# zhongzisha/multi_frame_super_resolution

Measured on AMD Instinct MI355X. Metric: Mpix/s end-to-end (N-frame burst -> x2 SR), higher is better.
Workload: dtype f32

## Files before the change

### include/mfsr.h

```cpp
#ifndef MFSR_H
#define MFSR_H

#include <stddef.h>
#include <stdint.h>

#ifdef __cplusplus
extern "C" {
#endif

#define MFSR_VERSION 100
#define MFSR_MAX_FUSE_GROUP 4

typedef void* mfsr_stream_t;

typedef struct { float x, y; } mfsr_float2;
typedef struct { float x, y, z; } mfsr_float3;
typedef struct { float x, y, z, w; } mfsr_float4;

typedef struct {
    const void* ptr;
    int32_t pitch;
    int32_t width;
    int32_t height;
} mfsr_tex2d;
// ... 228 lines not shown
                                    const float* movedImg, int pitchImg, const float* sumIn, const float* diffIn, float* sumOut,
                                    float* diffOut, int pitchSD, int width, int height, int halfWindowSize, float minDet,
                                    float outScale, mfsr_stream_t stream);
typedef struct {
    const uint16_t* dataIn;
    mfsr_float3* halfOut;
    float* pyr0;
    float* pyr1;
} mfsr_prepare_frame;
int mfsr_prepareFrameFusedBatch(int nFrames, const mfsr_prepare_frame* frames, int halfPitch, float maxVal, int dimX, int dimY,
                                int pyr0Pitch, int pyr1Pitch, const float* taps, int ntaps, mfsr_stream_t stream);
typedef struct {
    const float* movedImg;
    const mfsr_float2* coarseShifts;
    mfsr_float2* coordinates;
    const mfsr_prealign* base;
} mfsr_track_frame;
int mfsr_trackTilesFastSupported(int tileSize, int maxShift);
int mfsr_trackTilesFusedBatch(int nFrames, const mfsr_track_frame* frames, const float* refImg, int coarsePitch, int oldLevel,
                              int newLevel, int oldCountX, int oldCountY, int oldTileSize, int coordinatesPitch, int imgWidth,
                              int imgHeight, int imgPitch, int maxShift, int tileSize, int tileCountX, int tileCountY, float threshold,
                              const float* refSquaredSums, float baseInvScale, mfsr_stream_t stream);
typedef struct {
    mfsr_float2* outImg;
    const mfsr_float2* tileShifts;
    const mfsr_prealign* base;
    const float* movedImg;
    float* sumOut;
    float* diffOut;
} mfsr_flowfield_frame;
int mfsr_CreateFlowFieldWarpedBatch(int nFrames, const mfsr_flowfield_frame* frames, int tilePitch, int tileCountX, int tileCountY,
                                    int imgWidth, int imgHeight, int imgPitch, const float* refImg, int pitchImg, int pitchSD,
                                    mfsr_stream_t stream);
typedef struct {
    const mfsr_float3* movedHalf;
    mfsr_float4* mask;
    const mfsr_float2* flow;
} mfsr_robustness_frame;
int mfsr_robustnessMaskFusedBatch(int nFrames, const mfsr_robustness_frame* frames, const mfsr_float3* rawImgRef, int flowPitch,
                                  int flowWidth, int flowHeight, int imgWidth, int imgHeight, int imgPitch, int maskPitch, float alpha,
                                  float beta, float thresholdM, mfsr_stream_t stream);
typedef struct {
    const mfsr_float2* shiftsIn;
    mfsr_float2* shiftsOut;
    const float* movedImg;
    const float* sumIn;
    const float* diffIn;
    float* sumOut;
    float* diffOut;
} mfsr_lk_frame;
int mfsr_lucasKanadeSweepBatch(int nFrames, const mfsr_lk_frame* frames, const float* refImg, int pitchShift, int pitchImg,
                               int pitchSD, int width, int height, int halfWindowSize, float minDet, float outScale,
                               mfsr_stream_t stream);
int mfsr_CreateFlowFieldWarped(mfsr_float2* outImg, mfsr_tex2d texObjShiftXY, int imgWidth, int imgHeight, int imgPitch,
                               mfsr_float2 baseShift, float baseRotation, const mfsr_prealign* base, const float* refImg,
                               const float* movedImg, int pitchImg, float* sumOut, float* diffOut, int pitchSD,
                               mfsr_stream_t stream);

int mfsr_finishFusedRows(const mfsr_float3* finalImg, const mfsr_float3* weight, int imgPitch, const mfsr_float3* fallback,
                         int fbPitch, int fbW, int fbH, float u0, float u1, float v0, float v1, mfsr_float3* outImg,
                         int outPitch, uint16_t* out16, int width, int height, float threshold, int applyGamma, float maxOut,
                         int rowOffset, int fullHeight, mfsr_stream_t stream);
int mfsr_finishFusedWindow(const mfsr_float3* finalImg, const mfsr_float3* weight, int imgPitch, const mfsr_float3* fallback,
                           int fbPitch, int fbW, int fbH, float u0, float u1, float v0, float v1, mfsr_float3* outImg,
                           int outPitch, uint16_t* out16, int width, int height, float threshold, int applyGamma, float maxOut,
                           int colOffset, int rowOffset, int fullWidth, int fullHeight, mfsr_stream_t stream);

typedef struct {
    int32_t width, height;
    int32_t frames;
    int32_t reference;
    int32_t scale;
    int32_t mono;
    int32_t cfa[4];
    float black[3], white[3];
    float maxVal;
    int32_t levels;
    int32_t levelFactor[4];
    int32_t tileSize[4];
    int32_t maxShift[4];
    float minimumThreshold;
    float sigmaTracking;
    int32_t lkIterations;
    int32_t lkHalfWindow;
    float lkMinDet;
    float alpha, beta, thresholdM;
    float sigmaTensor;
    float Dth, Dtr, kDetail, kDenoise, kStretch, kShrink;
    float weightThreshold;
    int32_t applyGamma;
    int32_t fused;
    int32_t pairFrames;
    int32_t asyncFuse;
    int32_t preAlign;
    float preAlignMaxAngle;
    int32_t uploadRing;
    int32_t reserved[2];
} mfsr_config;

typedef struct mfsr_burst mfsr_burst;

int mfsr_config_default(mfsr_config* cfg, int width, int height, int frames, int scale, int mono);
size_t mfsr_burst_workspace_bytes(const mfsr_config* cfg);
size_t mfsr_burst_accumulator_bytes(const mfsr_config* cfg);
int mfsr_burst_create(mfsr_burst** out, const mfsr_config* cfg, void* workspace, size_t workspaceBytes);
void mfsr_burst_destroy(mfsr_burst* b);
// ... 87 lines not shown
```

### multi_frame_super_resolution_amd/csrc/lk_fused.hip

```cpp
#include <cstdlib>
#include <cstring>
#include "common.hpp"
#include "lk_math.hpp"

#ifndef LK_TY
#define LK_TY 16
#endif

__device__ __forceinline__ int lk_mirror_index(int i, int n)
{
    i = i < 0 ? -1 - i : i;
    return i >= n ? 2 * n - 1 - i : i;
}

template <typename T>
__device__ __forceinline__ T* lk_at(T* base, int pitch, int y, int x)
{
    return (T*)((char*)base + (uint32_t)((uint32_t)y * (uint32_t)pitch + (uint32_t)x * (uint32_t)sizeof(T)));
}

__device__ __forceinline__ void lk_warp_sample(const float* __restrict__ refImg, const float* __restrict__ movedImg, int pitchImg,
                                               int width, int height, int gx, int gy, float2 f, float& wv, float& rv,
                                               const MfsrExactDiv* dW = nullptr, const MfsrExactDiv* dH = nullptr)
{
// ... 231 lines not shown
            }                                                                                                          \
        }                                                                                                              \
        hipLaunchKernelGGL((k_lkIterationFused<HT, TXV, PRE>), grid, block, lds, mfsr_s(stream), (const float2*)shiftsIn, \
                           (float2*)shiftsOut, pitchShift, refImg, movedImg, pitchImg, width, height, h, minDet,       \
                           outScale, sumIn, diffIn, sumOut, diffOut, pitchSD);                                         \
    } while (0)
#define LK_CASE(HT)                                                                                                    \
    case HT:                                                                                                           \
        if (PRE && TX == 64)                                                                                           \
            LK_LAUNCH(HT, 64);                                                                                         \
        else if (TX == 48)                                                                                             \
            LK_LAUNCH(HT, 48);                                                                                         \
        else                                                                                                           \
            LK_LAUNCH(HT, 32);                                                                                         \
        break;
    switch (h) {
        LK_CASE(1)
        LK_CASE(2)
        LK_CASE(3)
        LK_CASE(4)
        LK_CASE(5)
        LK_CASE(6)
        LK_CASE(7)
        default:
            if (TX != 32) return MFSR_E_UNSUPPORTED;
            LK_LAUNCH(0, 32);
            break;
    }
#undef LK_CASE
#undef LK_LAUNCH
    return mfsr_launch_status("lucasKanadeIterationFused");
}

extern "C" int mfsr_lucasKanadeIterationFused(const mfsr_float2* shiftsIn, mfsr_float2* shiftsOut, int pitchShift,
                                              const float* refImg, const float* movedImg, int pitchImg, int width,
                                              int height, int halfWindowSize, float minDet, float outScale, mfsr_stream_t stream)
{
    return lk_iteration_impl<false>(shiftsIn, shiftsOut, pitchShift, refImg, movedImg, pitchImg, width, height, halfWindowSize, minDet,
                                    outScale, nullptr, nullptr, nullptr, nullptr, 0, stream);
}

extern "C" int mfsr_lucasKanadeIterationWarped(const mfsr_float2* shiftsIn, mfsr_float2* shiftsOut, int pitchShift,
                                               const float* refImg, const float* movedImg, int pitchImg, const float* sumIn,
                                               const float* diffIn, float* sumOut, float* diffOut, int pitchSD, int width, int height,
                                               int halfWindowSize, float minDet, float outScale, mfsr_stream_t stream)
{
    MFSR_REQUIRE(sumIn && diffIn && (sumOut != nullptr) == (diffOut != nullptr) && sumOut != sumIn && diffOut != diffIn);
    MFSR_REQUIRE((long long)pitchSD >= 4LL * width && (pitchSD & 3) == 0);
    MFSR_REQUIRE(!sumOut || outScale == 1.0f);
    return lk_iteration_impl<true>(shiftsIn, shiftsOut, pitchShift, refImg, movedImg, pitchImg, width, height, halfWindowSize, minDet,
                                   outScale, sumIn, diffIn, sumOut, diffOut, pitchSD, stream);
}

template <bool BASE_PTR>
__global__ void __launch_bounds__(256)
    k_flowFieldWarped(float2* __restrict__ outImg, mfsr_tex2d texShift, int imgWidth, int imgHeight, int imgPitch, float2 baseShift,
                      float baseRotation, const mfsr_prealign* __restrict__ base, const float* __restrict__ refImg,
                      const float* __restrict__ movedImg, int pitchImg, float* __restrict__ sumOut, float* __restrict__ diffOut,
                      int pitchSD, MfsrBatch bt, MfsrExactDiv dW, MfsrExactDiv dH)
{
    if (gridDim.z > 1) {
        outImg = (float2*)bt.p[blockIdx.z][0];
        texShift.ptr = bt.p[blockIdx.z][1];
        base = (const mfsr_prealign*)bt.p[blockIdx.z][2];
        movedImg = (const float*)bt.p[blockIdx.z][3];
        sumOut = (float*)bt.p[blockIdx.z][4];
        diffOut = (float*)bt.p[blockIdx.z][5];
    }
    const int pxX = blockIdx.x * blockDim.x + threadIdx.x;
    const int pxY = blockIdx.y * blockDim.y + threadIdx.y;
    if (pxX >= imgWidth || pxY >= imgHeight) return;
    float cf = 1.0f, sf = 0.0f, bx, by;
    if (BASE_PTR) {
        cf = base->cosRotation;
        sf = base->sinRotation;
        bx = base->shiftX;
        by = base->shiftY;
    } else {
        if (baseRotation != 0.0f) {
            cf = cosf(baseRotation);
            sf = sinf(baseRotation);
        }
        bx = baseShift.x;
        by = baseShift.y;
    }
    float2 shift;
    shift.x = cf * -bx - sf * -by;
    shift.y = sf * -bx + cf * -by;
    const float patchCenterX = (float)(pxX - imgWidth / 2);
    const float patchCenterY = (float)(pxY - imgHeight / 2);
    shift.x += cf * patchCenterX - sf * patchCenterY - patchCenterX;
    shift.y += sf * patchCenterX + cf * patchCenterY - patchCenterY;
    const float2 shiftPatch =
        tex2<ADDR_CLAMP>(texShift, mfsr_div((float)pxX + 0.5f, dW), mfsr_div((float)pxY + 0.5f, dH));
    shift.x += shiftPatch.x;
    shift.y += shiftPatch.y;
    *lk_at(outImg, imgPitch, pxY, pxX) = shift;
    float wv, rv;
    lk_warp_sample(refImg, movedImg, pitchImg, imgWidth, imgHeight, pxX, pxY, shift, wv, rv, &dW, &dH);
    *lk_at(sumOut, pitchSD, pxY, pxX) = wv + rv;
    *lk_at(diffOut, pitchSD, pxY, pxX) = wv - rv;
}

static int flow_field_warped_impl(int n, const mfsr_flowfield_frame* f, int tilePitch, int tileW, int tileH, int imgWidth, int imgHeight,
                                  int imgPitch, mfsr_float2 baseShift, float baseRotation, const float* refImg, int pitchImg, int pitchSD,
                                  mfsr_stream_t stream)
{
    MFSR_REQUIRE(f && n >= 1 && n <= MFSR_BATCH_MAX && refImg && imgWidth >= 2 && imgHeight >= 2);
    MFSR_REQUIRE((long long)imgPitch >= 8LL * imgWidth && (imgPitch & 7) == 0);
    MFSR_REQUIRE((long long)pitchImg >= 4LL * imgWidth && (pitchImg & 3) == 0 && (long long)pitchSD >= 4LL * imgWidth && (pitchSD & 3) == 0);
    if ((long long)imgPitch * imgHeight >= (1LL << 32) || (long long)pitchImg * imgHeight >= (1LL << 32) ||
        (long long)pitchSD * imgHeight >= (1LL << 32))
        return MFSR_E_UNSUPPORTED;
    mfsr_tex2d tex;
    tex.ptr = f[0].tileShifts;
    tex.pitch = tilePitch;
    tex.width = tileW;
    tex.height = tileH;
    MFSR_REQUIRE(mfsr_tex_ok(tex, 8) && (tilePitch & 7) == 0);
    MfsrBatch bt;
    memset(&bt, 0, sizeof(bt));
    for (int i = 0; i < n; i++) {
        MFSR_REQUIRE(f[i].outImg && f[i].tileShifts && f[i].movedImg && f[i].sumOut && f[i].diffOut);
        MFSR_REQUIRE(((uintptr_t)f[i].outImg & 7) == 0 && ((uintptr_t)f[i].tileShifts & 7) == 0);
        MFSR_REQUIRE((f[i].base != nullptr) == (f[0].base != nullptr));
        bt.p[i][0] = f[i].outImg;
        bt.p[i][1] = f[i].tileShifts;
        bt.p[i][2] = f[i].base;
        bt.p[i][3] = f[i].movedImg;
        bt.p[i][4] = f[i].sumOut;
        bt.p[i][5] = f[i].diffOut;
    }
    dim3 block(64, 4), grid(mfsr_cdiv(imgWidth, 64), mfsr_cdiv(imgHeight, 4), n);
    const MfsrExactDiv dW = mfsr_exact_div((float)imgWidth), dH = mfsr_exact_div((float)imgHeight);
    if (f[0].base)
        hipLaunchKernelGGL(k_flowFieldWarped<true>, grid, block, 0, mfsr_s(stream), (float2*)f[0].outImg, tex, imgWidth, imgHeight, imgPitch,
                           make_float2(0.0f, 0.0f), 0.0f, f[0].base, refImg, f[0].movedImg, pitchImg, f[0].sumOut, f[0].diffOut, pitchSD, bt, dW, dH);
    else
        hipLaunchKernelGGL(k_flowFieldWarped<false>, grid, block, 0, mfsr_s(stream), (float2*)f[0].outImg, tex, imgWidth, imgHeight, imgPitch,
                           make_float2(baseShift.x, baseShift.y), baseRotation, f[0].base, refImg, f[0].movedImg, pitchImg, f[0].sumOut,
                           f[0].diffOut, pitchSD, bt, dW, dH);
    return mfsr_launch_status("CreateFlowFieldWarped");
}

extern "C" int mfsr_CreateFlowFieldWarped(mfsr_float2* outImg, mfsr_tex2d texObjShiftXY, int imgWidth, int imgHeight, int imgPitch,
                                          mfsr_float2 baseShift, float baseRotation, const mfsr_prealign* base, const float* refImg,
                                          const float* movedImg, int pitchImg, float* sumOut, float* diffOut, int pitchSD,
                                          mfsr_stream_t stream)
{
    const mfsr_flowfield_frame f = {outImg, (const mfsr_float2*)texObjShiftXY.ptr, base, movedImg, sumOut, diffOut};
    return flow_field_warped_impl(1, &f, texObjShiftXY.pitch, texObjShiftXY.width, texObjShiftXY.height, imgWidth, imgHeight, imgPitch,
                                  baseShift, baseRotation, refImg, pitchImg, pitchSD, stream);
}

extern "C" int mfsr_CreateFlowFieldWarpedBatch(int nFrames, const mfsr_flowfield_frame* frames, int tilePitch, int tileCountX,
                                               int tileCountY, int imgWidth, int imgHeight, int imgPitch, const float* refImg,
                                               int pitchImg, int pitchSD, mfsr_stream_t stream)
{
    const mfsr_float2 z = {0.0f, 0.0f};
    return flow_field_warped_impl(nFrames, frames, tilePitch, tileCountX, tileCountY, imgWidth, imgHeight, imgPitch, z, 0.0f, refImg,
                                  pitchImg, pitchSD, stream);
}

#define MFSR_LK_SWEEP_MAX_BATCH 4
struct LkSweepFrame {
    const float2* flowIn;
    float2* flowOut;
    const float* moved;
    const float* sumIn;
    const float* diffIn;
    float* sumOut;
    float* diffOut;
};
struct LkSweepBatch {
    LkSweepFrame f[MFSR_LK_SWEEP_MAX_BATCH];
};

__device__ __forceinline__ float lk_wshr1(float v)
{
    return __uint_as_float(__builtin_amdgcn_update_dpp(0u, __float_as_uint(v), 0x138, 0xf, 0xf, true));
}
__device__ __forceinline__ float lk_wshl1(float v)
{
    return __uint_as_float(__builtin_amdgcn_update_dpp(0u, __float_as_uint(v), 0x130, 0xf, 0xf, true));
}

#ifndef LK_RV_REREAD
#define LK_RV_REREAD 0
#endif
#ifndef LK_DIFF_LATE
#define LK_DIFF_LATE 1
#endif
struct LkGather {
    float t00, t10, t01, t11, a, b;
#if !LK_RV_REREAD
    float rv;
#endif
};
__device__ __forceinline__ void lk_warp_issue(const float* __restrict__ movedImg, int pitchImg, int width, int height, int gx, int gy,
                                              float2 f, bool wanted, LkGather& g, const MfsrExactDiv& dW, const MfsrExactDiv& dH)
{
    const float u = mfsr_div((float)gx + 0.5f + f.x, dW);
    const float v = mfsr_div((float)gy + 0.5f + f.y, dH);
    const float xB = u * (float)width - 0.5f, yB = v * (float)height - 0.5f;
    const float fx = floorf(xB), fy = floorf(yB);
    const int ix = f2i(fx), iy = f2i(fy);
    const bool interior = u >= 0.0f && u < 1.0f && v >= 0.0f && v < 1.0f && (uint32_t)ix <= (uint32_t)(width - 2) &&
                          (uint32_t)iy <= (uint32_t)(height - 2);
    const int ixc = clampi(ix, 0, width - 2), iyc = clampi(iy, 0, height - 2);
    const float* r0 = lk_at(movedImg, pitchImg, iyc, ixc);
    const float* r1 = lk_at(movedImg, pitchImg, iyc + 1, ixc);
    g.t00 = r0[0], g.t10 = r0[1], g.t01 = r1[0], g.t11 = r1[1];
    g.a = xB - fx, g.b = yB - fy;
    if (__ballot(!interior && wanted) != 0) {
        mfsr_tex2d texMoved;
        texMoved.ptr = movedImg;
        texMoved.pitch = pitchImg;
        texMoved.width = width;
        texMoved.height = height;
        const float full = tex1<ADDR_MIRROR>(texMoved, u, v);
        if (!interior) {
            g.t00 = g.t10 = g.t01 = g.t11 = full;
            g.a = g.b = 0.0f;
        }
    }
}
__device__ __forceinline__ float lk_warp_finish(const LkGather& g) { return lerp4(g.t00, g.t10, g.t01, g.t11, g.a, g.b); }

template <int HT>
__global__ void __launch_bounds__(64)
    k_lkSweep(LkSweepBatch batch, const float* __restrict__ refImg, int pitchShift, int pitchImg, int pitchSD, int width, int height,
              float minDet, float outScale, int bandRows, int strips, int bands, int perXcd, int nFramesLaunch, MfsrExactDiv dW, MfsrExactDiv dH)
{
    constexpr int h = HT, HALO = HT + 2, WIN = 2 * HT + 1, VW = 64 - 2 * HALO;
    int sIdx, bIdx, fIdx;
    if (perXcd > 0) {
        const int t = ((int)blockIdx.x & 7) * perXcd + ((int)blockIdx.x >> 3);
        if (t >= strips * bands * nFramesLaunch) return;
        sIdx = t % strips;
        bIdx = (t / strips) % bands;
        fIdx = t / (strips * bands);
    } else {
        sIdx = blockIdx.x, bIdx = blockIdx.y, fIdx = blockIdx.z;
    }
    const LkSweepFrame F = batch.f[fIdx];
    const int lane = threadIdx.x;
    const int cx0 = sIdx * VW, ry0 = bIdx * bandRows;
    const int colIn = cx0 - HALO + lane;
    const int gxIn = lk_mirror_index(colIn, width);
    const int colOut = colIn - h;
    const bool outLane = lane >= 2 * h + 2 && lane <= 61 && colOut < width;
    const int colOutC = min(max(colOut, 0), width - 1);
    const bool ringCol = colOut < h || colOut >= width - h;
    const int rows = min(bandRows, height - ry0);
    const int T = rows + 2 * HALO;

    float s0 = 0, s1 = 0, s2 = 0, s3 = 0, s4 = 0;
    float d0 = 0;
    float H[5][WIN];
#pragma unroll
    for (int k = 0; k < 5; k++)
#pragma unroll
        for (int j = 0; j < WIN; j++) H[k][j] = 0.0f;

    auto load_sum = [&](int t, float& sv) { sv = *lk_at(F.sumIn, pitchSD, lk_mirror_index(ry0 - HALO + t, height), gxIn); };
    auto load_diff = [&](int t, float& dv) { dv = *lk_at(F.diffIn, pitchSD, lk_mirror_index(ry0 - HALO + t, height), gxIn); };
    float sA, sB, dA = 0, dB = 0;
    load_sum(0, sA);
    load_sum(min(1, T - 1), sB);
#if !LK_DIFF_LATE
    float d1 = 0, d2 = 0;
    load_diff(0, dA);
    load_diff(min(1, T - 1), dB);
#endif
    LkGather pend;
    int pendY = -1;
    auto finish_pending = [&]() {
        if (pendY < 0) return;
        const float wv = lk_warp_finish(pend);
#if LK_RV_REREAD
        const float rv = *lk_at(refImg, pitchImg, pendY, colOutC);
#else
        const float rv = pend.rv;
#endif
        if (outLane) {
            *lk_at(F.sumOut, pitchSD, pendY, colOutC) = wv + rv;
            *lk_at(F.diffOut, pitchSD, pendY, colOutC) = wv - rv;
        }
    };

    for (int t0 = 0; t0 < T; t0 += WIN) {
#pragma unroll
        for (int j = 0; j < WIN; j++) {
            const int t = t0 + j;
            if (t >= T) break;
            s0 = s1, s1 = s2, s2 = s3, s3 = s4, s4 = sA;
#if LK_DIFF_LATE
            d0 = dA, dA = dB;
            sA = sB;
            load_sum(min(t + 2, T - 1), sB);
            load_diff(t, dB);
#else
            d0 = d1, d1 = d2, d2 = dA, dA = dB;
            sA = sB;
            load_sum(min(t + 2, T - 1), sB);
            load_diff(min(t + 2, T - 1), dB);
#endif
            if (t < 4) continue;
            const int y = ry0 + t - 2 * HALO;
            const int yc = min(max(y, 0), height - 1);
            float2 shift = *lk_at(F.flowIn, pitchShift, yc, colOutC);
#if !LK_RV_REREAD
            const float rvOwn = *lk_at(refImg, pitchImg, yc, colOutC);
#endif
            const float xp1 = lk_wshl1(s2), xp2 = lk_wshl1(xp1), xm1 = lk_wshr1(s2), xm2 = lk_wshr1(xm1);
            float tx = xp2;
            tx -= xp1 * 8.0f;
            tx += xm1 * 8.0f;
            tx -= xm2;
            const float Ix = tx * (1.0f / 24.0f);
            float ty = s4;
            ty -= s3 * 8.0f;
            ty += s1 * 8.0f;
            ty -= s0;
            const float Iy = ty * (1.0f / 24.0f);
            const float It = d0;
            float P[5] = {Ix * Ix, Ix * Iy, Iy * Iy, Ix * It, Iy * It};
#pragma unroll
            for (int k = 0; k < 5; k++) {
                float acc = P[k];
#pragma unroll
                for (int q = 0; q < 2 * HT; q++) acc = P[k] + lk_wshr1(acc);
                H[k][j] = acc;
            }
            if (t < 2 * HALO) continue;
            float V[5];
#pragma unroll
            for (int k = 0; k < 5; k++) {
                float sum = 0;
#pragma unroll
                for (int d = 1; d <= WIN; d++) sum += H[k][(j + d) % WIN];
                V[k] = sum;
            }
            if (!(ringCol || y < h || y >= height - h)) {
                float inv[4];
                if (lk_pinv(V[0], V[1], V[2], minDet, inv)) {
                    float UV0 = inv[0] * V[3] + inv[1] * V[4];
                    float UV1 = inv[2] * V[3] + inv[3] * V[4];
                    UV0 = isnan(UV0) ? 0 : UV0;
                    UV1 = isnan(UV1) ? 0 : UV1;
                    shift.x += UV0;
                    shift.y += UV1;
                }
            }
            if (F.sumOut) {
                finish_pending();
                lk_warp_issue(F.moved, pitchImg, width, height, colOutC, y, shift, outLane, pend, dW, dH);
#if !LK_RV_REREAD
                pend.rv = rvOwn;
#endif
                pendY = y;
            }
            shift.x *= outScale;
            shift.y *= outScale;
            if (outLane) *lk_at(F.flowOut, pitchShift, y, colOutC) = shift;
        }
    }
    if (F.sumOut) finish_pending();
}

extern "C" int mfsr_lucasKanadeSweepBatch(int nFrames, const mfsr_lk_frame* frames, const float* refImg, int pitchShift, int pitchImg,
                                          int pitchSD, int width, int height, int halfWindowSize, float minDet, float outScale,
                                          mfsr_stream_t stream)
{
    MFSR_REQUIRE(frames && refImg && nFrames >= 1 && nFrames <= MFSR_LK_SWEEP_MAX_BATCH);
    if (halfWindowSize < 1 || halfWindowSize > 7 || width < 64 || height < 2 * (halfWindowSize + 2)) return MFSR_E_UNSUPPORTED;
    MFSR_REQUIRE((long long)pitchShift >= 8LL * width && (pitchShift & 7) == 0);
    MFSR_REQUIRE((long long)pitchImg >= 4LL * width && (pitchImg & 3) == 0 && (long long)pitchSD >= 4LL * width && (pitchSD & 3) == 0);
    if ((long long)pitchShift * height >= (1LL << 32) || (long long)pitchImg * height >= (1LL << 32) || (long long)pitchSD * height >= (1LL << 32))
        return MFSR_E_UNSUPPORTED;
    LkSweepBatch b;
    memset(&b, 0, sizeof(b));
    for (int i = 0; i < nFrames; i++) {
        const mfsr_lk_frame& f = frames[i];
        MFSR_REQUIRE(f.shiftsIn && f.shiftsOut && f.shiftsIn != f.shiftsOut && f.movedImg && f.sumIn && f.diffIn);
        MFSR_REQUIRE(((uintptr_t)f.shiftsIn & 7) == 0 && ((uintptr_t)f.shiftsOut & 7) == 0);
        MFSR_REQUIRE((f.sumOut != nullptr) == (f.diffOut != nullptr) && f.sumOut != f.sumIn && f.diffOut != f.diffIn);
        MFSR_REQUIRE(!f.sumOut || outScale == 1.0f);
        b.f[i] = LkSweepFrame{(const float2*)f.shiftsIn, (float2*)f.shiftsOut, f.movedImg, f.sumIn, f.diffIn, f.sumOut, f.diffOut};
    }
    const int h = halfWindowSize, VW = 64 - 2 * (h + 2);
    const int strips = mfsr_cdiv(width, VW);
    static const int forceBand = [] {
        const char* e = getenv("MFSR_LK_BAND");
        return e ? atoi(e) : 0;
    }();
    int band = (int)((long long)height * strips * nFrames / 8192);
    band = (band + 4) & ~7;
    band = band < 8 ? 8 : (band > 32 ? 32 : band);
    {
        static const int occ[8] = {0, 8, 7, 6, 5, 4, 4, 4};
        const long long places = 1024LL * occ[h];
        const long long maxBands = places / ((long long)strips * nFrames);
        if (maxBands >= 1) {
            int b = (int)((height + maxBands - 1) / maxBands);
            b = b < 8 ? 8 : b;
            if (b <= 64) band = b;
        }
    }
    if (forceBand >= 8) band = forceBand;
    static const int xcdRemap = [] {
        const char* e = getenv("MFSR_LK_XCD");
        return e ? atoi(e) : 1;
    }();
    const int bands = mfsr_cdiv(height, band);
    const int total = strips * bands * nFrames;
    const int perXcd = xcdRemap ? mfsr_cdiv(total, 8) : 0;
    dim3 grid = perXcd ? dim3(8 * perXcd, 1, 1) : dim3(strips, bands, nFrames), block(64);
    const MfsrExactDiv dW = mfsr_exact_div((float)width), dH = mfsr_exact_div((float)height);
#define LKS_CASE(HT)                                                                                                          \
    case HT:                                                                                                                  \
        hipLaunchKernelGGL(k_lkSweep<HT>, grid, block, 0, mfsr_s(stream), b, refImg, pitchShift, pitchImg, pitchSD, width,    \
                           height, minDet, outScale, band, strips, bands, perXcd, nFrames, dW, dH);                           \
        break;
    switch (h) {
        LKS_CASE(1)
        LKS_CASE(2)
        LKS_CASE(3)
        LKS_CASE(4)
        LKS_CASE(5)
        LKS_CASE(6)
        LKS_CASE(7)
    }
#undef LKS_CASE
    return mfsr_launch_status("lucasKanadeSweepBatch");
}
```

### multi_frame_super_resolution_amd/csrc/pipeline.cpp

```cpp
#include <hip/hip_runtime.h>

#include <cstdio>
#include <cstring>
#include <new>
#include <utility>
#include <vector>

#include "common.hpp"

namespace {

constexpr int kMaxLevels = 4;
constexpr int kMaxTimedLaunches = 4096;
constexpr int kRing = 2 * MFSR_MAX_FUSE_GROUP;
constexpr int kMaxUploadRing = 32;

inline size_t align_up(size_t v, size_t a) { return (v + a - 1) / a * a; }

struct Img {
    void* ptr = nullptr;
    int pitch = 0;
    int w = 0, h = 0;
};

// ... 1051 lines not shown
            TRY(mfsr_zeroRing_f32x4((mfsr_float4*)mask->ptr, mask->pitch, L.hw, L.hh, stream));
            TRY(mfsr_ComputeRobustnessMask((const mfsr_float3*)L.refHalf.ptr, (const mfsr_float3*)L.movHalf.ptr,
                                           (mfsr_float4*)mask->ptr, as_tex(*flow), L.hw, L.hh, L.refHalf.pitch, mask->pitch,
                                           c.alpha, c.beta, c.thresholdM, stream));
        }
      }
    }
    *flowOut = flow;
    *maskOut = mask;
    b->slotFlow[slot] = flow;
    return MFSR_OK;
}

static bool can_defer_alignment(const mfsr_burst* b)
{
    static const bool on = [] {
        const char* e = getenv("MFSR_ALIGN_BATCH");
        return !(e && e[0] == '0');
    }();
    const mfsr_config& c = b->cfg;
    static const bool hostDefer = [] {
        const char* e = getenv("MFSR_HOST_DEFER");
        return e && e[0] == '1';
    }();
    const bool hostImmediate = b->holdLastGroup && !b->hostBusy && (b->framesSinceRef < b->group || !hostDefer);
    return on && b->group > 1 && b->L.nSets >= b->group - 1 && lk_warped_path(b) && c.lkHalfWindow >= 1 && c.lkHalfWindow <= 7 &&
           !b->movPrepared && !b->givenShifts && !hostImmediate;
}

static int align_deferred(mfsr_burst* b, mfsr_stream_t stream)
{
    const mfsr_config& c = b->cfg;
    Layout& L = b->L;
    int idx[MFSR_MAX_FUSE_GROUP], n = 0;
    for (int i = 0; i < b->pend.n; i++)
        if (b->pend.deferred[i]) idx[n++] = i;
    if (n == 0) return MFSR_OK;
    TRY(wait_uploads(b, stream));
    auto movHalf = [&](int q) -> Img& { return q == 0 ? L.movHalf : L.sets[q - 1].movHalf; };
    auto movPyr = [&](int q) -> Img* { return q == 0 ? L.movPyr : L.sets[q - 1].movPyr; };
    auto shiftsOf = [&](int q) -> Img* { return q == 0 ? L.shifts : L.sets[q - 1].shifts; };
    auto lkSumOf = [&](int q) -> Img* { return q == 0 ? L.lkSum : L.sets[q - 1].lkSum; };
    auto lkDiffOf = [&](int q) -> Img* { return q == 0 ? L.lkDiff : L.sets[q - 1].lkDiff; };
    static const bool stageBatchOn = [] {
        const char* e = getenv("MFSR_ALIGN_BATCH");
        return !(e && e[0] == '1' && e[1] == 's');
    }();
    const int nlev = ilog2(L.maxFactor) + 1;
    bool stageBatch = stageBatchOn && c.fused && !c.mono && !c.preAlign && b->ntaps / 2 <= 8 && L.tw == L.hw && L.th == L.hh;
    for (int l = 0; l < c.levels && stageBatch; l++) stageBatch = mfsr_trackTilesFastSupported(c.tileSize[l], c.maxShift[l]) != 0;
    int mq[MFSR_MAX_FUSE_GROUP], m = 0;
    for (int q = 0; q < n; q++)
        if (!b->pend.isRef[idx[q]]) mq[m++] = q;
    if (stageBatch) {
        for (int q = 0; q < n; q++) {
            const int i = idx[q], slot = b->pend.slot[i];
            if (b->pend.isRef[i]) {
                Img *flow = nullptr, *mask = nullptr;
                TRY(align_frame(b, b->pend.raw[i], 1, slot, &flow, &mask, stream, ALIGN_PRE));
            } else if (b->fuseStream && b->fusedOutstanding[slot]) {
                MFSR_HIP_TRY(hipStreamWaitEvent(mfsr_s(stream), b->evFused[slot], 0));
                b->fusedOutstanding[slot] = false;
            }
        }
        if (m > 0) {
            TRY(mfsr_set_cfa_pattern(c.cfa));
            mfsr_prepare_frame pf[MFSR_MAX_FUSE_GROUP];
            for (int k = 0; k < m; k++) {
                Img* pyr = movPyr(mq[k]);
                pf[k].dataIn = b->pend.raw[idx[mq[k]]];
                pf[k].halfOut = (mfsr_float3*)movHalf(mq[k]).ptr;
                pf[k].pyr0 = (float*)pyr[0].ptr;
                pf[k].pyr1 = nlev > 1 ? (float*)pyr[1].ptr : nullptr;
            }
            TRY(mfsr_prepareFrameFusedBatch(m, pf, L.movHalf.pitch, c.maxVal, L.hw, L.hh, L.movPyr[0].pitch, nlev > 1 ? L.movPyr[1].pitch : 0,
                                            b->taps, b->ntaps, stream));
            for (int k = 0; k < m; k++) {
                Img* pyr = movPyr(mq[k]);
                for (int i = 2; i < nlev; i++)
                    TRY(mfsr_downsample2x((const float*)pyr[i - 1].ptr, pyr[i - 1].pitch, (float*)pyr[i].ptr, pyr[i].pitch, pyr[i].w, pyr[i].h,
                                          stream));
            }
            for (int l = 0; l < c.levels; l++) {
                const int pi = ilog2(c.levelFactor[l]);
                mfsr_track_frame tf[MFSR_MAX_FUSE_GROUP];
                for (int k = 0; k < m; k++) {
                    tf[k].movedImg = (const float*)movPyr(mq[k])[pi].ptr;
                    tf[k].coarseShifts = l > 0 ? (const mfsr_float2*)shiftsOf(mq[k])[l - 1].ptr : nullptr;
                    tf[k].coordinates = (mfsr_float2*)shiftsOf(mq[k])[l].ptr;
                    tf[k].base = nullptr;
                }
                const Img& ref = L.refPyr[pi];
                TRY(mfsr_trackTilesFusedBatch(m, tf, (const float*)ref.ptr, l > 0 ? L.shifts[l - 1].pitch : 0, l > 0 ? c.levelFactor[l - 1] : 0,
                                              c.levelFactor[l], l > 0 ? L.tcx[l - 1] : 0, l > 0 ? L.tcy[l - 1] : 0,
                                              l > 0 ? c.tileSize[l - 1] : 0, L.shifts[l].pitch, ref.w, ref.h, ref.pitch, c.maxShift[l],
                                              c.tileSize[l], L.tcx[l], L.tcy[l], c.minimumThreshold, L.refSq[l],
                                              1.0f / (float)c.levelFactor[l], stream));
            }
            const int last = c.levels - 1;
            mfsr_flowfield_frame ff[MFSR_MAX_FUSE_GROUP];
            for (int k = 0; k < m; k++) {
                const int slot = b->pend.slot[idx[mq[k]]];
                ff[k].outImg = (mfsr_float2*)L.flowBuf[2 * slot].ptr;
                ff[k].tileShifts = (const mfsr_float2*)shiftsOf(mq[k])[last].ptr;
                ff[k].base = nullptr;
                ff[k].movedImg = (const float*)movPyr(mq[k])[0].ptr;
                ff[k].sumOut = (float*)lkSumOf(mq[k])[0].ptr;
                ff[k].diffOut = (float*)lkDiffOf(mq[k])[0].ptr;
            }
            TRY(mfsr_CreateFlowFieldWarpedBatch(m, ff, L.shifts[last].pitch, L.shifts[last].w, L.shifts[last].h, L.tw, L.th,
                                                L.flowBuf[0].pitch, (const float*)L.refPyr[0].ptr, L.refPyr[0].pitch, L.lkSum[0].pitch, stream));
        }
    } else {
    for (int q = 0; q < n; q++) {
        const int i = idx[q];
        if (q > 0) swap_set(L, L.sets[q - 1]);
        Img *flow = nullptr, *mask = nullptr;
        const int rc = align_frame(b, b->pend.raw[i], b->pend.isRef[i], b->pend.slot[i], &flow, &mask, stream, ALIGN_PRE);
        if (q > 0) swap_set(L, L.sets[q - 1]);
        if (rc) return rc;
    }
    }
    bool batched = true;
    for (int it = 0; it < c.lkIterations && batched; it++) {
        mfsr_lk_frame fr[MFSR_MAX_FUSE_GROUP];
        int m = 0;
        const bool lastIt = it == c.lkIterations - 1;
        const int in = it & 1, out = in ^ 1;
        for (int q = 0; q < n; q++) {
            const int i = idx[q];
            if (b->pend.isRef[i]) continue;
            const int slot = b->pend.slot[i];
            const Img* sum = q == 0 ? L.lkSum : L.sets[q - 1].lkSum;
            const Img* diff = q == 0 ? L.lkDiff : L.sets[q - 1].lkDiff;
            const Img& mov = q == 0 ? L.movPyr[0] : L.sets[q - 1].movPyr[0];
            fr[m].shiftsIn = (const mfsr_float2*)L.flowBuf[2 * slot + in].ptr;
            fr[m].shiftsOut = (mfsr_float2*)L.flowBuf[2 * slot + out].ptr;
            fr[m].movedImg = (const float*)mov.ptr;
            fr[m].sumIn = (const float*)sum[in].ptr;
            fr[m].diffIn = (const float*)diff[in].ptr;
            fr[m].sumOut = lastIt ? nullptr : (float*)sum[out].ptr;
            fr[m].diffOut = lastIt ? nullptr : (float*)diff[out].ptr;
            m++;
        }
        if (m == 0) break;
        const int rc = mfsr_lucasKanadeSweepBatch(m, fr, (const float*)L.refPyr[0].ptr, L.flowBuf[0].pitch, L.refPyr[0].pitch,
                                                  L.lkSum[0].pitch, L.tw, L.th, c.lkHalfWindow, c.lkMinDet,
                                                  lastIt ? (float)L.flowScale : 1.0f, stream);
        if (rc == MFSR_E_UNSUPPORTED && it == 0)
            batched = false;
        else if (rc)
            return rc;
    }
    bool maskBatch = stageBatch && batched && m > 0;
    if (maskBatch) {
        mfsr_robustness_frame rf[MFSR_MAX_FUSE_GROUP];
        for (int k = 0; k < m; k++) {
            const int slot = b->pend.slot[idx[mq[k]]];
            rf[k].movedHalf = (const mfsr_float3*)movHalf(mq[k]).ptr;
            rf[k].mask = (mfsr_float4*)L.maskBuf[slot].ptr;
            rf[k].flow = (const mfsr_float2*)L.flowBuf[2 * slot + (c.lkIterations & 1)].ptr;
        }
        const int rc = mfsr_robustnessMaskFusedBatch(m, rf, (const mfsr_float3*)L.refHalf.ptr, L.flowBuf[0].pitch, L.tw, L.th, L.hw, L.hh,
                                                     L.refHalf.pitch, L.maskBuf[0].pitch, c.alpha, c.beta, c.thresholdM, stream);
        if (rc == MFSR_E_UNSUPPORTED)
            maskBatch = false;
        else if (rc)
            return rc;
    }
    for (int q = 0; q < n; q++) {
        const int i = idx[q];
        if (q > 0) swap_set(L, L.sets[q - 1]);
        Img *flow = nullptr, *mask = nullptr;
        const int rc = align_frame(b, b->pend.raw[i], b->pend.isRef[i], b->pend.slot[i], &flow, &mask, stream,
                                   maskBatch ? 0 : (batched ? ALIGN_POST : (ALIGN_LK | ALIGN_POST)));
        if (q > 0) swap_set(L, L.sets[q - 1]);
        if (rc) return rc;
        b->pend.flow[i] = flow;
        b->pend.mask[i] = mask;
        b->pend.deferred[i] = false;
        b->flowCur = flow;
        b->maskCur = mask;
        if (b->fuseStream) MFSR_HIP_TRY(hipEventRecord(b->evAligned[b->pend.slot[i]], mfsr_s(stream)));
    }
    return MFSR_OK;
}

static int add_frame_impl(mfsr_burst* b, const uint16_t* raw, int isReference, mfsr_float3* imgOut, mfsr_float3* totalWeights,
                          bool hostBurst, mfsr_stream_t stream)
{
    MFSR_REQUIRE(b && raw && imgOut && totalWeights);
    MFSR_REQUIRE(b->haveRef);
    MFSR_REQUIRE(!b->refStale);
    const mfsr_config& c = b->cfg;
    TRY(mfsr_set_cfa_pattern(c.cfa));
    b->holdLastGroup = hostBurst;
    if (b->pend.n && (b->pend.imgOut != imgOut || b->pend.totalWeights != totalWeights)) TRY(flush_pending(b, stream));
    if (b->pend.n >= b->group) TRY(accumulate_pending(b, stream));
    MFSR_REQUIRE(b->pend.n < MFSR_MAX_FUSE_GROUP);
    const int slot = b->frameCounter++ % kRing;
    Img *flow = nullptr, *mask = nullptr;
    const bool defer = can_defer_alignment(b);
// ... 1128 lines not shown
```

Before: 22550.

## Fuse flow-field creation into the first Lucas-Kanade sweep iteration

Adds a first-iteration variant of the LK sweep kernel. It computes the per-pixel flow directly from the tile shifts using bilinear interpolation, warps the moved image inline, and forms the sum and difference values on the fly, keeping the flow for each row in a shared-memory ring. The pipeline skips the separate flow-field-warped kernel when this path is on (the default, controlled by an environment variable). This removes one launch and the global write and re-read of the flow, sum and difference images. In exchange the first sweep does more work per thread and uses a lower-occupancy band plan, and an unsupported-shape return from the fused path becomes an error instead of falling back.

```diff
diff --git a/include/mfsr.h b/include/mfsr.h
--- a/include/mfsr.h
+++ b/include/mfsr.h
@@ -304,6 +304,9 @@
 int mfsr_lucasKanadeSweepBatch(int nFrames, const mfsr_lk_frame* frames, const float* refImg, int pitchShift, int pitchImg,
                                int pitchSD, int width, int height, int halfWindowSize, float minDet, float outScale,
                                mfsr_stream_t stream);
+int mfsr_lucasKanadeSweepFromTilesBatch(int nFrames, const mfsr_lk_frame* frames, int tilePitch, int tileCountX, int tileCountY,
+                                        const float* refImg, int pitchShift, int pitchImg, int pitchSD, int width, int height,
+                                        int halfWindowSize, float minDet, float outScale, mfsr_stream_t stream);
 int mfsr_CreateFlowFieldWarped(mfsr_float2* outImg, mfsr_tex2d texObjShiftXY, int imgWidth, int imgHeight, int imgPitch,
                                mfsr_float2 baseShift, float baseRotation, const mfsr_prealign* base, const float* refImg,
                                const float* movedImg, int pitchImg, float* sumOut, float* diffOut, int pitchSD,
diff --git a/multi_frame_super_resolution_amd/csrc/lk_fused.hip b/multi_frame_super_resolution_amd/csrc/lk_fused.hip
--- a/multi_frame_super_resolution_amd/csrc/lk_fused.hip
+++ b/multi_frame_super_resolution_amd/csrc/lk_fused.hip
@@ -307,6 +307,33 @@
                                    outScale, sumIn, diffIn, sumOut, diffOut, pitchSD, stream);
 }
 
+template <bool OFF32 = false>
+__device__ __forceinline__ float2 lk_flow_field_at(const mfsr_tex2d& texShift, int pxX, int pxY, int imgWidth, int imgHeight, float cf,
+                                                   float sf, float bx, float by, const MfsrExactDiv& dW, const MfsrExactDiv& dH)
+{
+    float2 shift;
+    shift.x = cf * -bx - sf * -by;
+    shift.y = sf * -bx + cf * -by;
+    const float patchCenterX = (float)(pxX - imgWidth / 2);
+    const float patchCenterY = (float)(pxY - imgHeight / 2);
+    shift.x += cf * patchCenterX - sf * patchCenterY - patchCenterX;
+    shift.y += sf * patchCenterX + cf * patchCenterY - patchCenterY;
+    const float tu = mfsr_div((float)pxX + 0.5f, dW), tv = mfsr_div((float)pxY + 0.5f, dH);
+    float2 shiftPatch;
+    if (OFF32) {
+        const TexCoord c = tex_coord<ADDR_CLAMP>(texShift.width, texShift.height, tu, tv);
+        const float2* tp = (const float2*)texShift.ptr;
+        const float2 t00 = *lk_at(tp, texShift.pitch, c.j0, c.i0), t10 = *lk_at(tp, texShift.pitch, c.j0, c.i1);
+        const float2 t01 = *lk_at(tp, texShift.pitch, c.j1, c.i0), t11 = *lk_at(tp, texShift.pitch, c.j1, c.i1);
+        shiftPatch = make_float2(lerp4(t00.x, t10.x, t01.x, t11.x, c.a, c.b), lerp4(t00.y, t10.y, t01.y, t11.y, c.a, c.b));
+    } else {
+        shiftPatch = tex2<ADDR_CLAMP>(texShift, tu, tv);
+    }
+    shift.x += shiftPatch.x;
+    shift.y += shiftPatch.y;
+    return shift;
+}
+
 template <bool BASE_PTR>
 __global__ void __launch_bounds__(256)
     k_flowFieldWarped(float2* __restrict__ outImg, mfsr_tex2d texShift, int imgWidth, int imgHeight, int imgPitch, float2 baseShift,
@@ -339,17 +366,7 @@
         bx = baseShift.x;
         by = baseShift.y;
     }
-    float2 shift;
-    shift.x = cf * -bx - sf * -by;
-    shift.y = sf * -bx + cf * -by;
-    const float patchCenterX = (float)(pxX - imgWidth / 2);
-    const float patchCenterY = (float)(pxY - imgHeight / 2);
-    shift.x += cf * patchCenterX - sf * patchCenterY - patchCenterX;
-    shift.y += sf * patchCenterX + cf * patchCenterY - patchCenterY;
-    const float2 shiftPatch =
-        tex2<ADDR_CLAMP>(texShift, mfsr_div((float)pxX + 0.5f, dW), mfsr_div((float)pxY + 0.5f, dH));
-    shift.x += shiftPatch.x;
-    shift.y += shiftPatch.y;
+    const float2 shift = lk_flow_field_at(texShift, pxX, pxY, imgWidth, imgHeight, cf, sf, bx, by, dW, dH);
     *lk_at(outImg, imgPitch, pxY, pxX) = shift;
     float wv, rv;
     lk_warp_sample(refImg, movedImg, pitchImg, imgWidth, imgHeight, pxX, pxY, shift, wv, rv, &dW, &dH);
@@ -430,6 +447,9 @@
 struct LkSweepBatch {
     LkSweepFrame f[MFSR_LK_SWEEP_MAX_BATCH];
 };
+struct LkTiles {
+    int pitch, w, h;
+};
 
 __device__ __forceinline__ float lk_wshr1(float v)
 {
@@ -482,10 +502,11 @@
 }
 __device__ __forceinline__ float lk_warp_finish(const LkGather& g) { return lerp4(g.t00, g.t10, g.t01, g.t11, g.a, g.b); }
 
-template <int HT>
+template <int HT, bool FIRST = false>
 __global__ void __launch_bounds__(64)
     k_lkSweep(LkSweepBatch batch, const float* __restrict__ refImg, int pitchShift, int pitchImg, int pitchSD, int width, int height,
-              float minDet, float outScale, int bandRows, int strips, int bands, int perXcd, int nFramesLaunch, MfsrExactDiv dW, MfsrExactDiv dH)
+              float minDet, float outScale, int bandRows, int strips, int bands, int perXcd, int nFramesLaunch, MfsrExactDiv dW, MfsrExactDiv dH,
+              LkTiles tiles)
 {
     constexpr int h = HT, HALO = HT + 2, WIN = 2 * HT + 1, VW = 64 - 2 * HALO;
     int sIdx, bIdx, fIdx;
@@ -520,9 +541,33 @@
 
     auto load_sum = [&](int t, float& sv) { sv = *lk_at(F.sumIn, pitchSD, lk_mirror_index(ry0 - HALO + t, height), gxIn); };
     auto load_diff = [&](int t, float& dv) { dv = *lk_at(F.diffIn, pitchSD, lk_mirror_index(ry0 - HALO + t, height), gxIn); };
-    float sA, sB, dA = 0, dB = 0;
-    load_sum(0, sA);
-    load_sum(min(1, T - 1), sB);
+    float sA = 0, sB = 0, dA = 0, dB = 0;
+    mfsr_tex2d texTiles;
+    texTiles.ptr = F.flowIn;
+    texTiles.pitch = tiles.pitch;
+    texTiles.width = tiles.w;
+    texTiles.height = tiles.h;
+    auto flow_at = [&](int gx, int gy) { return lk_flow_field_at<true>(texTiles, gx, gy, width, height, 1.0f, 0.0f, 0.0f, 0.0f, dW, dH); };
+    constexpr int LK_FLOW_RING = HALO + 2 <= 8 ? 8 : 16;
+    static_assert(LK_FLOW_RING >= HALO + 2, "the ring holds the rows between an input row's warp issue and its output step");
+    __shared__ float2 s_flow[FIRST ? LK_FLOW_RING : 1][64];
+    const int laneFrom = max(lane - h, 0);
+    LkGather gA;
+    float rA = 0;
+    auto issue_in = [&](int t, LkGather& g, float& rv) {
+        const int gy = lk_mirror_index(ry0 - HALO + t, height);
+        const float2 f = flow_at(gxIn, gy);
+        if (FIRST) s_flow[t % LK_FLOW_RING][lane] = f;
+        lk_warp_issue(F.moved, pitchImg, width, height, gxIn, gy, f, true, g, dW, dH);
+        rv = *lk_at(refImg, pitchImg, gy, gxIn);
+    };
+    static_assert(LK_DIFF_LATE || !FIRST, "the first-iteration sweep keeps the LK_DIFF_LATE difference ring");
+    if (FIRST) {
+        issue_in(0, gA, rA);
+    } else {
+        load_sum(0, sA);
+        load_sum(min(1, T - 1), sB);
+    }
 #if !LK_DIFF_LATE
     float d1 = 0, d2 = 0;
     load_diff(0, dA);
@@ -549,22 +594,29 @@
         for (int j = 0; j < WIN; j++) {
             const int t = t0 + j;
             if (t >= T) break;
-            s0 = s1, s1 = s2, s2 = s3, s3 = s4, s4 = sA;
+            if (FIRST) {
+                const float wv = lk_warp_finish(gA);
+                s0 = s1, s1 = s2, s2 = s3, s3 = s4, s4 = wv + rA;
+                d0 = dA, dA = dB, dB = wv - rA;
+                issue_in(min(t + 1, T - 1), gA, rA);
+            } else {
+                s0 = s1, s1 = s2, s2 = s3, s3 = s4, s4 = sA;
 #if LK_DIFF_LATE
-            d0 = dA, dA = dB;
-            sA = sB;
-            load_sum(min(t + 2, T - 1), sB);
-            load_diff(t, dB);
+                d0 = dA, dA = dB;
+                sA = sB;
+                load_sum(min(t + 2, T - 1), sB);
+                load_diff(t, dB);
 #else
-            d0 = d1, d1 = d2, d2 = dA, dA = dB;
-            sA = sB;
-            load_sum(min(t + 2, T - 1), sB);
-            load_diff(min(t + 2, T - 1), dB);
-#endif
+                d0 = d1, d1 = d2, d2 = dA, dA = dB;
+                sA = sB;
+                load_sum(min(t + 2, T - 1), sB);
+                load_diff(min(t + 2, T - 1), dB);
+#endif
+            }
             if (t < 4) continue;
             const int y = ry0 + t - 2 * HALO;
             const int yc = min(max(y, 0), height - 1);
-            float2 shift = *lk_at(F.flowIn, pitchShift, yc, colOutC);
+            float2 shift = FIRST ? s_flow[(t - HALO) % LK_FLOW_RING][laneFrom] : *lk_at(F.flowIn, pitchShift, yc, colOutC);
 #if !LK_RV_REREAD
             const float rvOwn = *lk_at(refImg, pitchImg, yc, colOutC);
 #endif
@@ -624,11 +676,13 @@
     if (F.sumOut) finish_pending();
 }
 
-extern "C" int mfsr_lucasKanadeSweepBatch(int nFrames, const mfsr_lk_frame* frames, const float* refImg, int pitchShift, int pitchImg,
-                                          int pitchSD, int width, int height, int halfWindowSize, float minDet, float outScale,
-                                          mfsr_stream_t stream)
+static int lk_sweep_impl(int nFrames, const mfsr_lk_frame* frames, bool first, LkTiles tiles, const float* refImg, int pitchShift,
+                         int pitchImg, int pitchSD, int width, int height, int halfWindowSize, float minDet, float outScale,
+                         mfsr_stream_t stream)
 {
     MFSR_REQUIRE(frames && refImg && nFrames >= 1 && nFrames <= MFSR_LK_SWEEP_MAX_BATCH);
+    MFSR_REQUIRE(!first || (tiles.w > 0 && tiles.h > 0 && (long long)tiles.pitch >= 8LL * tiles.w && (tiles.pitch & 7) == 0));
+    if (first && (long long)tiles.pitch * tiles.h >= (1LL << 32)) return MFSR_E_UNSUPPORTED;
     if (halfWindowSize < 1 || halfWindowSize > 7 || width < 64 || height < 2 * (halfWindowSize + 2)) return MFSR_E_UNSUPPORTED;
     MFSR_REQUIRE((long long)pitchShift >= 8LL * width && (pitchShift & 7) == 0);
     MFSR_REQUIRE((long long)pitchImg >= 4LL * width && (pitchImg & 3) == 0 && (long long)pitchSD >= 4LL * width && (pitchSD & 3) == 0);
@@ -638,11 +692,12 @@
     memset(&b, 0, sizeof(b));
     for (int i = 0; i < nFrames; i++) {
         const mfsr_lk_frame& f = frames[i];
-        MFSR_REQUIRE(f.shiftsIn && f.shiftsOut && f.shiftsIn != f.shiftsOut && f.movedImg && f.sumIn && f.diffIn);
+        MFSR_REQUIRE(f.shiftsIn && f.shiftsOut && f.shiftsIn != f.shiftsOut && f.movedImg && (first || (f.sumIn && f.diffIn)));
         MFSR_REQUIRE(((uintptr_t)f.shiftsIn & 7) == 0 && ((uintptr_t)f.shiftsOut & 7) == 0);
-        MFSR_REQUIRE((f.sumOut != nullptr) == (f.diffOut != nullptr) && f.sumOut != f.sumIn && f.diffOut != f.diffIn);
+        MFSR_REQUIRE((f.sumOut != nullptr) == (f.diffOut != nullptr) && (!f.sumOut || (f.sumOut != f.sumIn && f.diffOut != f.diffIn)));
         MFSR_REQUIRE(!f.sumOut || outScale == 1.0f);
-        b.f[i] = LkSweepFrame{(const float2*)f.shiftsIn, (float2*)f.shiftsOut, f.movedImg, f.sumIn, f.diffIn, f.sumOut, f.diffOut};
+        b.f[i] = LkSweepFrame{(const float2*)f.shiftsIn, (float2*)f.shiftsOut, f.movedImg, first ? nullptr : f.sumIn,
+                              first ? nullptr : f.diffIn, f.sumOut, f.diffOut};
     }
     const int h = halfWindowSize, VW = 64 - 2 * (h + 2);
     const int strips = mfsr_cdiv(width, VW);
@@ -655,7 +710,8 @@
     band = band < 8 ? 8 : (band > 32 ? 32 : band);
     {
         static const int occ[8] = {0, 8, 7, 6, 5, 4, 4, 4};
-        const long long places = 1024LL * occ[h];
+        static const int occFirst[8] = {0, 6, 5, 5, 4, 4, 4, 3};
+        const long long places = 1024LL * (first ? occFirst[h] : occ[h]);
         const long long maxBands = places / ((long long)strips * nFrames);
         if (maxBands >= 1) {
             int b = (int)((height + maxBands - 1) / maxBands);
@@ -675,8 +731,12 @@
     const MfsrExactDiv dW = mfsr_exact_div((float)width), dH = mfsr_exact_div((float)height);
 #define LKS_CASE(HT)                                                                                                          \
     case HT:                                                                                                                  \
-        hipLaunchKernelGGL(k_lkSweep<HT>, grid, block, 0, mfsr_s(stream), b, refImg, pitchShift, pitchImg, pitchSD, width,    \
-                           height, minDet, outScale, band, strips, bands, perXcd, nFrames, dW, dH);                           \
+        if (first)                                                                                                            \
+            hipLaunchKernelGGL((k_lkSweep<HT, true>), grid, block, 0, mfsr_s(stream), b, refImg, pitchShift, pitchImg, pitchSD, \
+                               width, height, minDet, outScale, band, strips, bands, perXcd, nFrames, dW, dH, tiles);         \
+        else                                                                                                                  \
+            hipLaunchKernelGGL((k_lkSweep<HT, false>), grid, block, 0, mfsr_s(stream), b, refImg, pitchShift, pitchImg, pitchSD, \
+                               width, height, minDet, outScale, band, strips, bands, perXcd, nFrames, dW, dH, tiles);         \
         break;
     switch (h) {
         LKS_CASE(1)
@@ -688,5 +748,21 @@
         LKS_CASE(7)
     }
 #undef LKS_CASE
-    return mfsr_launch_status("lucasKanadeSweepBatch");
-}
+    return mfsr_launch_status(first ? "lucasKanadeSweepFromTilesBatch" : "lucasKanadeSweepBatch");
+}
+
+extern "C" int mfsr_lucasKanadeSweepBatch(int nFrames, const mfsr_lk_frame* frames, const float* refImg, int pitchShift, int pitchImg,
+                                          int pitchSD, int width, int height, int halfWindowSize, float minDet, float outScale,
+                                          mfsr_stream_t stream)
+{
+    return lk_sweep_impl(nFrames, frames, false, LkTiles{0, 0, 0}, refImg, pitchShift, pitchImg, pitchSD, width, height, halfWindowSize,
+                         minDet, outScale, stream);
+}
+
+extern "C" int mfsr_lucasKanadeSweepFromTilesBatch(int nFrames, const mfsr_lk_frame* frames, int tilePitch, int tileCountX, int tileCountY,
+                                                   const float* refImg, int pitchShift, int pitchImg, int pitchSD, int width, int height,
+                                                   int halfWindowSize, float minDet, float outScale, mfsr_stream_t stream)
+{
+    return lk_sweep_impl(nFrames, frames, true, LkTiles{tilePitch, tileCountX, tileCountY}, refImg, pitchShift, pitchImg, pitchSD, width,
+                         height, halfWindowSize, minDet, outScale, stream);
+}
diff --git a/multi_frame_super_resolution_amd/csrc/pipeline.cpp b/multi_frame_super_resolution_amd/csrc/pipeline.cpp
--- a/multi_frame_super_resolution_amd/csrc/pipeline.cpp
+++ b/multi_frame_super_resolution_amd/csrc/pipeline.cpp
@@ -1127,6 +1127,12 @@
     int mq[MFSR_MAX_FUSE_GROUP], m = 0;
     for (int q = 0; q < n; q++)
         if (!b->pend.isRef[idx[q]]) mq[m++] = q;
+    static const bool fusedEndsOn = [] {
+        const char* e = getenv("MFSR_LK_FUSED_ENDS");
+        return !(e && e[0] == '0');
+    }();
+    const bool fusedFirst = fusedEndsOn && stageBatch && m > 0;
+    const int last = c.levels - 1;
     if (stageBatch) {
         for (int q = 0; q < n; q++) {
             const int i = idx[q], slot = b->pend.slot[i];
@@ -1172,7 +1178,6 @@
                                               c.tileSize[l], L.tcx[l], L.tcy[l], c.minimumThreshold, L.refSq[l],
                                               1.0f / (float)c.levelFactor[l], stream));
             }
-            const int last = c.levels - 1;
             mfsr_flowfield_frame ff[MFSR_MAX_FUSE_GROUP];
             for (int k = 0; k < m; k++) {
                 const int slot = b->pend.slot[idx[mq[k]]];
@@ -1183,8 +1188,10 @@
                 ff[k].sumOut = (float*)lkSumOf(mq[k])[0].ptr;
                 ff[k].diffOut = (float*)lkDiffOf(mq[k])[0].ptr;
             }
-            TRY(mfsr_CreateFlowFieldWarpedBatch(m, ff, L.shifts[last].pitch, L.shifts[last].w, L.shifts[last].h, L.tw, L.th,
-                                                L.flowBuf[0].pitch, (const float*)L.refPyr[0].ptr, L.refPyr[0].pitch, L.lkSum[0].pitch, stream));
+            if (!fusedFirst)
+                TRY(mfsr_CreateFlowFieldWarpedBatch(m, ff, L.shifts[last].pitch, L.shifts[last].w, L.shifts[last].h, L.tw, L.th,
+                                                    L.flowBuf[0].pitch, (const float*)L.refPyr[0].ptr, L.refPyr[0].pitch, L.lkSum[0].pitch,
+                                                    stream));
         }
     } else {
     for (int q = 0; q < n; q++) {
@@ -1201,6 +1208,7 @@
         mfsr_lk_frame fr[MFSR_MAX_FUSE_GROUP];
         int m = 0;
         const bool lastIt = it == c.lkIterations - 1;
+        const bool fromTiles = fusedFirst && it == 0;
         const int in = it & 1, out = in ^ 1;
         for (int q = 0; q < n; q++) {
             const int i = idx[q];
@@ -1209,7 +1217,7 @@
             const Img* sum = q == 0 ? L.lkSum : L.sets[q - 1].lkSum;
             const Img* diff = q == 0 ? L.lkDiff : L.sets[q - 1].lkDiff;
             const Img& mov = q == 0 ? L.movPyr[0] : L.sets[q - 1].movPyr[0];
-            fr[m].shiftsIn = (const mfsr_float2*)L.flowBuf[2 * slot + in].ptr;
+            fr[m].shiftsIn = fromTiles ? (const mfsr_float2*)shiftsOf(q)[last].ptr : (const mfsr_float2*)L.flowBuf[2 * slot + in].ptr;
             fr[m].shiftsOut = (mfsr_float2*)L.flowBuf[2 * slot + out].ptr;
             fr[m].movedImg = (const float*)mov.ptr;
             fr[m].sumIn = (const float*)sum[in].ptr;
@@ -1219,10 +1227,14 @@
             m++;
         }
         if (m == 0) break;
-        const int rc = mfsr_lucasKanadeSweepBatch(m, fr, (const float*)L.refPyr[0].ptr, L.flowBuf[0].pitch, L.refPyr[0].pitch,
-                                                  L.lkSum[0].pitch, L.tw, L.th, c.lkHalfWindow, c.lkMinDet,
-                                                  lastIt ? (float)L.flowScale : 1.0f, stream);
-        if (rc == MFSR_E_UNSUPPORTED && it == 0)
+        const float outScale = lastIt ? (float)L.flowScale : 1.0f;
+        const int rc = fromTiles
+                           ? mfsr_lucasKanadeSweepFromTilesBatch(m, fr, L.shifts[last].pitch, L.shifts[last].w, L.shifts[last].h,
+                                                                 (const float*)L.refPyr[0].ptr, L.flowBuf[0].pitch, L.refPyr[0].pitch,
+                                                                 L.lkSum[0].pitch, L.tw, L.th, c.lkHalfWindow, c.lkMinDet, outScale, stream)
+                           : mfsr_lucasKanadeSweepBatch(m, fr, (const float*)L.refPyr[0].ptr, L.flowBuf[0].pitch, L.refPyr[0].pitch,
+                                                        L.lkSum[0].pitch, L.tw, L.th, c.lkHalfWindow, c.lkMinDet, outScale, stream);
+        if (rc == MFSR_E_UNSUPPORTED && it == 0 && !fromTiles)
             batched = false;
         else if (rc)
             return rc;
```

After: 22760, median of 6. About the same (+0.9%).
